# google/nerfies

Measured on NVIDIA H100. Metric: ray-samples/sec (coarse+fine, device-timed), higher is better.
Workload: dtype fp16x3 (fp32 emulated on wgmma: 3 fp16 MMA chains, fp32 accumulate)

## Files before the change

nerfies_b200/csrc/field_simt.cuh:

```cuda
#pragma once
#include "common.cuh"

namespace nfb {

constexpr int kTM = 64;
constexpr int kRS = kTM + 4;
constexpr int kKS = 16;
constexpr int kSimtThreads = 256;
constexpr int kSimtSmemFloats =
    2 * kMaxWidth * kRS
    + kMaxIn * kRS
    + 64 * kRS
    + 2 * kKS * kMaxWidth
    + 3 * kTM;
constexpr int kSimtSmemBytes = kSimtSmemFloats * 4;

constexpr int kDebugTimeout = 8, kDebugOneRowBlock = 16;

struct FieldArgs {
  const float* params;
  const float* origins;
  const float* directions;
  const float* z_vals;
  const float* points;
  const float* cond;
  const float* window;
  float* samples;
  float* warped;
  long long num_rows;
  int samples_per_ray;
  int use_warp;
  int warp_only;
  int debug;
  float* ray_out;
  float* ray_weights;
  int white_bg, sample_at_infinity;
};

__device__ __forceinline__ void cp_async16(void* smem, const void* gmem) {
  unsigned s = (unsigned)__cvta_generic_to_shared(smem);
  asm volatile("cp.async.cg.shared.global [%0], [%1], 16;\n" ::"r"(s), "l"(gmem));
}
__device__ __forceinline__ void cp_async_commit() {
  asm volatile("cp.async.commit_group;\n" ::);
}
template <int N>
__device__ __forceinline__ void cp_async_wait() {
  asm volatile("cp.async.wait_group %0;\n" ::"n"(N));
}

struct SimtSmem {
  float* buf[2];
  float* in;
  float* out;
  float* slab[2];
  float* wp;
  __device__ float* ptr(int id) const {
    return id == kB0 ? buf[0] : id == kB1 ? buf[1] : id == kOut0 ? out : out + 32 * kRS;
  }
// ... 189 lines not shown
```

nerfies_b200/csrc/field_tc.cuh:

```cuda
#pragma once
#include "field_simt.cuh"
#include "field_tc3.cuh"
#include "nfb_handle.h"
#include "tc_common.cuh"
#include "tc_program.cuh"

namespace nfb {
namespace tc {

__device__ __forceinline__ void posenc_fast_to_block(uint8_t* block, int r, const float* x, int F,
                                                  const float* __restrict__ window,
                                                  const float* __restrict__ extra, int n_extra,
                                                  int c_begin = 0, int c_end = 8) {
  float feat[64];
#pragma unroll
  for (int k = 0; k < 64; ++k) feat[k] = 0.f;
  float sn[3], cs[3];
#pragma unroll
  for (int c = 0; c < 3; ++c) {
    feat[c] = x[c];
    sincosf(x[c], &sn[c], &cs[c]);
  }
#pragma unroll
  for (int f = 0; f < 10; ++f) {
// ... 9 lines not shown
      }
    }
  }
  const int d = 3 + 6 * F;
#pragma unroll
  for (int k = 0; k < 64; ++k) {
    if (k >= d && k < d + n_extra) feat[k] = __ldg(extra + (k - d));
  }
#pragma unroll
  for (int c = 0; c < 8; ++c)
    if (c >= c_begin && c < c_end) store_chunk(block, r, c, feat + c * 8);
}
template <bool kX3, uint32_t kBlkBytes>
__device__ __forceinline__ void encode_input(uint8_t* in_block, int r, int hs, const float* x, int F,
                                             const float* __restrict__ window,
                                             const float* __restrict__ extra, int n_extra) {
  if constexpr (kX3) {
    if (hs == 0) tc3::posenc_block_x3<0>(in_block, in_block + kBlkBytes, r, x, F, window, extra, n_extra);
    else tc3::posenc_block_x3<1>(in_block, in_block + kBlkBytes, r, x, F, window, extra, n_extra);
  } else {
    posenc_fast_to_block(in_block, r, x, F, window, extra, n_extra, 4 * hs, 4 * hs + 4);
  }
}
__device__ __forceinline__ void cond_to_block(uint8_t* block, int r, const float* __restrict__ cond,
                                              int n, int c_begin = 0, int c_end = 8) {
#pragma unroll 1
  for (int c = c_begin; c < c_end; ++c) {
    float v[8];
#pragma unroll
    for (int j = 0; j < 8; ++j) {
      const int k = c * 8 + j;
      v[j] = k < n ? __ldg(cond + k) : 0.f;
    }
    store_chunk(block, r, c, v);
  }
}

template <bool kX3, uint32_t kBlkBytes>
__device__ __forceinline__ void epi_chunk(const float* acc, int c, const float* __restrict__ bias, float inv_s,
                                          bool relu, bool adot, const float* __restrict__ aw, float& al0,
                                          float& al1, uint8_t* act_hi, uint32_t* lo, int arow, int lq) {
#pragma unroll
  for (int j = 0; j < 16; ++j) {
    const int col = c * 128 + 8 * j + 2 * lq;
    const float2 b = __ldg(reinterpret_cast<const float2*>(bias + col));
    float v[4] = {fmaf(acc[4 * j], inv_s, b.x), fmaf(acc[4 * j + 1], inv_s, b.y),
                  fmaf(acc[4 * j + 2], inv_s, b.x), fmaf(acc[4 * j + 3], inv_s, b.y)};
    if (adot) {
      float2 w = __ldg(reinterpret_cast<const float2*>(aw + col));
      if constexpr (!kX3) w = __bfloat1622float2(__floats2bfloat162_rn(w.x, w.y));
      al0 = fmaf(relu ? fmaxf(v[0], 0.f) : v[0], w.x, al0);
      al0 = fmaf(relu ? fmaxf(v[1], 0.f) : v[1], w.y, al0);
      al1 = fmaf(relu ? fmaxf(v[2], 0.f) : v[2], w.x, al1);
      al1 = fmaf(relu ? fmaxf(v[3], 0.f) : v[3], w.y, al1);
    }
    const uint32_t blk = (uint32_t)(2 * c + (j >> 3)) * kBlkBytes + 4 * lq;
#pragma unroll
    for (int h = 0; h < 2; ++h) {
      const uint32_t off = blk + swz_off(arow + 8 * h, j & 7);
      const float a = v[2 * h], bb = v[2 * h + 1];
      uint32_t hi;
      if constexpr (kX3) {
        const float ta = __uint_as_float(__float_as_uint(a) & 0xFFFFE000u);
        const float tb = __uint_as_float(__float_as_uint(bb) & 0xFFFFE000u);
        const float da = a - ta, db = bb - tb;
        uint32_t& l = lo[x3_lo_reg(2 * c + (j >> 3), j & 7, h)];
        if (relu) {
          asm("cvt.rn.relu.satfinite.f16x2.f32 %0, %1, %2;" : "=r"(hi) : "f"(tb), "f"(ta));
          asm("cvt.rn.relu.satfinite.f16x2.f32 %0, %1, %2;" : "=r"(l) : "f"(db), "f"(da));
        } else {
          asm("cvt.rn.satfinite.f16x2.f32 %0, %1, %2;" : "=r"(hi) : "f"(tb), "f"(ta));
          asm("cvt.rn.satfinite.f16x2.f32 %0, %1, %2;" : "=r"(l) : "f"(db), "f"(da));
        }
      } else {
        if (relu) asm("cvt.rn.relu.bf16x2.f32 %0, %1, %2;" : "=r"(hi) : "f"(bb), "f"(a));
        else asm("cvt.rn.bf16x2.f32 %0, %1, %2;" : "=r"(hi) : "f"(bb), "f"(a));
      }
      *reinterpret_cast<uint32_t*>(act_hi + off) = hi;
    }
  }
}

template <bool kX3>
__device__ __noinline__ float alpha_cond_dot(const float* __restrict__ cond, const float* __restrict__ w, int n) {
  float a = 0.f;
  for (int j = 0; j < n; ++j) {
    float wj = __ldg(w + j);
    if constexpr (!kX3) wj = __bfloat162float(__float2bfloat16_rn(wj));
    a = fmaf(__ldg(cond + j), wj, a);
  }
  return a;
}

struct RowState {
  float x[3];
  long long m;
  long long ray;
  bool valid;
  float z, dist;
  bool last;
};

constexpr int kWgThreads = 384;
constexpr int kAlphaOff = 14 * kABlockBytes;
constexpr int kScanOff = kAlphaOff + 512;
constexpr int kBarOff = kScanOff + 256;
constexpr int kWgSmemBytes = kBarOff + 256;
template <bool kX3, int kMB>
struct WgSmem {
  static constexpr int kRows = kMB * kTileRows;
  static constexpr uint32_t kBlkBytes = kRows * kRowBytes;
  static constexpr int kSlots = (kX3 && kMB == 2) ? 3 : 4;
  static constexpr int kSlotBytes = (kX3 ? 2 : 1) * kABlockBytes;
  static constexpr int kRingOff = kAlphaOff - kSlots * kSlotBytes;
  static constexpr int kInOff = kRingOff - 2 * (int)kBlkBytes;
  static_assert(kInOff >= 4 * kABlockBytes, "input block overlaps the activation image");
};
static_assert(kWgSmemBytes <= 232448, "shared memory");

template <bool kX3, int N, int kActKb>
__device__ __forceinline__ void wg_layer_unit(float* d, int src, uint32_t a_hi, uint32_t in_lo, const uint32_t* lo,
                                              uint32_t b_hi, uint32_t b_lo, uint32_t accumulate) {
  if constexpr (kX3) {
    switch (src) {
      case 0: wg_unit<true, N>(d, a_hi, lo + x3_lo_reg(0, 0, 0), b_hi, b_lo, accumulate); break;
      case 1: wg_unit<true, N>(d, a_hi, lo + x3_lo_reg(1, 0, 0), b_hi, b_lo, accumulate); break;
      case 2:
        if constexpr (kActKb > 2) wg_unit<true, N>(d, a_hi, lo + x3_lo_reg(2, 0, 0), b_hi, b_lo, accumulate);
        break;
// ... 58 lines not shown
          const uint32_t bytes = (kX3 ? 2u : 1u) * (uint32_t)st.chunk_n * kRowBytes;
          const uint8_t* src = wpack + st.w_off;
          const int n = st.n_chunks * st.nkb;
          for (int u = 0; u < n; ++u) {
            mbar_wait(&bars->empty[sg], ph ^ 1, dead);
            if (!dead && elect_one()) {
              mbar_arrive_expect_tx(&bars->full[sg], bytes);
              bulk_g2s(ring + sg * kSlotBytes, src + (size_t)u * bytes, bytes, &bars->full[sg]);
            }
            __syncwarp();
            if (++sg == kSlots) { sg = 0; ph ^= 1; }
          }
        }
      }
    }
  } else {
    asm volatile("setmaxnreg.inc.sync.aligned.u32 %0;" ::"n"(kConsumerRegs));
    constexpr int kWgRows = 64 * kMB;
    const int cw = wg - 1, t = tid & 127, wq = t >> 5, lq = lane & 3;
    const int arow = kWgRows * cw + 16 * wq + (lane >> 2);
    const int lr = kMB == 2 ? t : (t & 63);
    const int r = kWgRows * cw + lr;
    const int h0 = kMB == 2 ? 0 : t >> 6, h1 = kMB == 2 ? 2 : h0 + 1;
    const int cb = h0 * 4, ce = cb + 4;
    uint8_t* act_hi = base;
    uint8_t* inh = base + Smem::kInOff;
    uint8_t* inl = inh + kBlk;
    float* alpha_s = reinterpret_cast<float*>(base + kAlphaOff);
    float* scan_s = reinterpret_cast<float*>(base + kScanOff);
    const uint32_t rows_off = (uint32_t)(kWgRows * cw * kRowBytes);
    float* scr = reinterpret_cast<float*>(base + rows_off);
    const uint32_t ring_a = smem_u32(base + Smem::kRingOff);
    const uint32_t act_a = smem_u32(act_hi) + rows_off, in_a = smem_u32(inh) + rows_off;
    uint32_t lo[kX3 ? 64 : 1];
    const float alpha_b = __ldg(aux + prog.alpha_b_off);
    const int S = args.samples_per_ray;
    uint32_t sg = 0, ph = 0, dead = 0;
    auto wg_sync = [&]() { asm volatile("bar.sync %0, 128;" ::"r"(1 + cw) : "memory"); };
    RowState row;

    auto begin_tile = [&](int tile) {
      long long m = (long long)tile * kRows + r;
      row.valid = m < args.num_rows;
      if (!row.valid) m = args.num_rows - 1;
      row.m = m;
      row.ray = m / S;
      const float z = args.z_vals ? __ldg(args.z_vals + m) : 0.f;
      float org[3], dir[3];
#pragma unroll
      for (int c = 0; c < 3; ++c) {
        dir[c] = __ldg(args.directions + row.ray * 3 + c);
        org[c] = __ldg(args.origins + row.ray * 3 + c);
      }
      if (args.points) {
#pragma unroll
        for (int c = 0; c < 3; ++c) row.x[c] = __ldg(args.points + m * 3 + c);
      } else {
#pragma unroll
        for (int c = 0; c < 3; ++c) row.x[c] = org[c] + z * dir[c];
      }
      if (fuse) {
        row.z = z;
        row.last = m + 1 == (row.ray + 1) * S;
        const float zn = (!row.last && args.z_vals) ? __ldg(args.z_vals + m + 1) : 0.f;
        const float dnorm = sqrtf(dir[0] * dir[0] + dir[1] * dir[1] + dir[2] * dir[2]);
        const float d = row.last ? (args.sample_at_infinity ? 1e10f : 1e-19f) : (zn - z);
        row.dist = d * dnorm;
      }
      if (!warp_pass && args.warped && row.valid && h0 == 0) {
// ... 41 lines not shown
            } else {
              wg_layer_unit<kX3, 128, kActKb>(acc0, src, a_hi, in_lo, lo, b_hi, b_lo, kb);
              wg_layer_unit<kX3, 128, kActKb>(acc1, src, a_hi + 8192u, in_lo + 8192u, lo + 32, b_hi, b_lo, kb);
            }
          }
          wg_commit();
          if (u > 0) {
            wg_wait<1>();
            if (lane == 0) mbar_arrive(&bars->empty[prev_sg]);
          }
          prev_sg = sg;
          if (++sg == kSlots) { sg = 0; ph ^= 1; }
        }
        wg_wait<0>();
        wg_fence_regs<64>(acc0); wg_fence_regs<64>(acc1);
        if (lane == 0) mbar_arrive(&bars->empty[prev_sg]);
        wg_sync();

        if (hidden) {
          const bool relu = st.relu != 0, adot = st.alpha_dot != 0;
          const float* aw = aux + prog.alpha_w_off;
          if constexpr (kMB == 1) {
            float al0 = 0.f, al1 = 0.f;
            epi_chunk<kX3, kBlk>(acc0, 0, bias, inv_s, relu, adot, aw, al0, al1, act_hi, lo, arow, lq);
            if (st.n_chunks == 2)
              epi_chunk<kX3, kBlk>(acc1, 1, bias, inv_s, relu, adot, aw, al0, al1, act_hi, lo, arow, lq);
            if (adot) {
              al0 += __shfl_xor_sync(0xffffffffu, al0, 1); al0 += __shfl_xor_sync(0xffffffffu, al0, 2);
              al1 += __shfl_xor_sync(0xffffffffu, al1, 1); al1 += __shfl_xor_sync(0xffffffffu, al1, 2);
              if (lq == 0) { alpha_s[arow] = al0; alpha_s[arow + 8] = al1; }
            }
            if (st.write_cond) {
              const float* cond = args.cond + row.ray * prog.cond_stride + prog.rc_off;
              if constexpr (kX3) tc3::cond_to_block_x3(inh, inl, r, cond, prog.rc, cb, ce);
              else cond_to_block(inh, r, cond, prog.rc, cb, ce);
            }
          } else {
            float al0 = 0.f, al1 = 0.f;
            epi_chunk<kX3, kBlk>(acc0, 0, bias, inv_s, relu, false, aw, al0, al1, act_hi, lo, arow, lq);
            epi_chunk<kX3, kBlk>(acc1, 0, bias, inv_s, relu, false, aw, al0, al1, act_hi, lo + 32, arow + 64, lq);
          }
        } else {
          const int l0 = 16 * wq + (lane >> 2);
#pragma unroll
          for (int b = 0; b < kMB; ++b) {
            const float* a16 = b == 0 ? acc0 : acc1;
#pragma unroll
            for (int h = 0; h < 2; ++h) {
              float* sr = scr + (l0 + 64 * b + 8 * h) * 16 + 2 * lq;
              sr[0] = a16[2 * h]; sr[1] = a16[2 * h + 1];
              sr[8] = a16[4 + 2 * h]; sr[9] = a16[5 + 2 * h];
            }
          }
          wg_sync();
          float v[12];
#pragma unroll
          for (int j = 0; j < 12; ++j) v[j] = fmaf(scr[lr * 16 + j], inv_s, __ldg(bias + j));
          wg_sync();
          if (st.epi == kEpiWarpHeads) {
            float y[3];
            warp_tail(prog.warp_type, v, row.x, prog.warp_pivot, prog.warp_trans, y);
            if (row.valid && h0 == 0) {
#pragma unroll
              for (int c = 0; c < 3; ++c) args.warped[row.m * 3 + c] = y[c];
            }
            if (has_next) begin_tile(tile_of(ti + 1));
          } else if constexpr (kMB == 1) {
            float4 o;
            o.x = sigmoidf(v[0]); o.y = sigmoidf(v[1]); o.z = sigmoidf(v[2]);
            const float a_cond = prog.ac ? alpha_cond_dot<kX3>(args.cond + row.ray * prog.cond_stride + prog.ac_off,
                                                               aux + prog.alpha_w_off + kAlphaCondOff, prog.ac)
                                         : 0.f;
            o.w = apply_act(alpha_b + (alpha_s[r] + a_cond), prog.sigma_act);
            if (h0 == 0 && row.valid && args.samples) reinterpret_cast<float4*>(args.samples)[row.m] = o;
            if (fuse && h0 == 0) {
              const int qd = r >> 5;
              auto bar128 = [&]() { asm volatile("bar.sync 3, 128;" ::: "memory"); };
              if ((tile % tpr) == 0) { c_T = 1.f; c_cw = 0.f; a_r = a_g = a_b = a_d = a_w = a_wnl = a_med = 0.f; }
              const float al = -expm1f(-o.w * row.dist);
              const float tf = 1.0f - al + 1e-10f;
              float P = tf;
#pragma unroll
              for (int sh = 1; sh < 32; sh <<= 1) {
                const float q = __shfl_up_sync(0xffffffffu, P, sh);
                if (lane >= sh) P = P * q;
              }
              float excl = __shfl_up_sync(0xffffffffu, P, 1);
              if (lane == 0) excl = 1.f;
              if (lane == 31) scan_s[qd] = P;
              bar128();
              float Wq = 1.f, Wall = 1.f;
#pragma unroll
              for (int q = 0; q < 4; ++q) {
                const float f = scan_s[q];
                if (q < qd) Wq = Wq * f;
                Wall = Wall * f;
// ... 43 lines not shown
                ro[5] = args.sample_at_infinity ? a_wnl : a_w;
              }
              bar128();
            }
            if (has_next) begin_tile(tile_of(ti + 1));
          }
          if constexpr (kX3) {
#pragma unroll
            for (int i = 0; i < 64; ++i) lo[i] = 0u;
          }
        }
        fence_proxy_async();
        wg_sync();
      }
    }
  }
  __syncthreads();
}

inline int tc_fail(const char* what) {
  return fail("the tensor-core paths (precision bf16 / fp16x3) do not support this model: %s; use precision fp32", what);
}

inline int build_tc_program(nfb_handle* h, int level, long long* wbytes, long long* aux_floats) {
  const FieldProgram& fp = h->prog[level];
  TcProgram& tp = h->tcprog[level];
  memset(&tp, 0, sizeof(tp));
  const int wparts = h->cfg.precision == NFB_PREC_FP16X3 ? 2 : 1;
  tp.warp_pivot = fp.warp_pivot; tp.warp_trans = fp.warp_trans;
  tp.warp_type = fp.warp_type; tp.Fw = fp.Fw; tp.G = fp.G; tp.Fp = fp.Fp; tp.rc = fp.rc;
  tp.cond_stride = fp.cond_stride; tp.sigma_act = fp.sigma_act;
  tp.tc = fp.tc; tp.ac = fp.ac; tp.ac_off = fp.G + fp.tc; tp.rc_off = fp.G + fp.tc + fp.ac;
  if (fp.rc > kBlockK) return tc_fail("rgb condition wider than 64 channels");
  if (fp.ac > kBlockK) return tc_fail("alpha condition wider than 64 channels");
  if (fp.Dp + fp.tc > kBlockK || (fp.warp_type && fp.Dw > kBlockK)) return tc_fail("encoded inputs wider than 64");
  if (fp.hidden_act != kRelu) return tc_fail("hidden activation other than relu");
  auto new_bias = [&](const Step& st) {
    int off = (int)*aux_floats;
    *aux_floats += 256;
    h->tc_aux_jobs.push_back({st.b_off, st.n, 1, off});
    return off;
  };
  auto add = [&](const Step& st, int epi, int cur_width) -> int {
    if (tp.n_steps >= kMaxTcSteps) return tc_fail("too many layers");
    TcStep& t = tp.steps[tp.n_steps];
    memset(&t, 0, sizeof(t));
    if (st.k_x > 256 || st.k_in > kBlockK) return tc_fail("layer wider than 256 or inputs wider than 64");
    if (st.k_x && st.k_x != cur_width) return tc_fail("unexpected layer input width");
    t.nkb = 0;
    if (st.k_in) t.src[t.nkb++] = kSrcIn;
    for (int b = 0; b < (st.k_x + kBlockK - 1) / kBlockK; ++b) t.src[t.nkb++] = b;
    t.epi = epi;
    if (epi == kEpiHidden) {
      if (st.n < 1 || st.n > 256) return tc_fail("hidden widths must be 1..256");
      t.n_chunks = (st.n + 127) / 128; t.chunk_n = 128;
      if (st.act != kRelu && st.act != kNone) return tc_fail("hidden activation other than relu");
      t.relu = st.act == kRelu;
    } else {
      t.n_chunks = 1; t.chunk_n = 16;
      if (st.n > 12) return tc_fail("head wider than 12");
      if (st.k_in) return tc_fail("head reading the encoded inputs");
    }
    t.b_off = new_bias(st);
    t.w_off = (uint32_t)*wbytes;
    for (int c = 0; c < t.n_chunks; ++c) {
      nfb_handle::TcPackJob job;
      job.level = level; job.step = tp.n_steps; job.chunk = c;
      job.simt_w_off = st.w_off; job.ld = st.npad; job.n = st.n; job.n0 = c * t.chunk_n;
      job.k_total = st.k_x + st.k_in;
      job.k_map.assign((size_t)t.nkb * kBlockK, -1);
      for (int kb = 0; kb < t.nkb; ++kb)
        for (int j = 0; j < kBlockK; ++j) {
          int srck = -1;
          if (t.src[kb] < kSrcIn) srck = t.src[kb] * kBlockK + j < st.k_x ? t.src[kb] * kBlockK + j : -1;
          else if (j < st.k_in) srck = st.k_x + j;
          job.k_map[(size_t)kb * kBlockK + j] = srck;
        }
      h->tc_jobs.push_back(job);
      *wbytes += (long long)wparts * t.nkb * t.chunk_n * kRowBytes;
    }
    ++tp.n_steps;
    return 0;
  };
  int width = 0;
  for (int i = 0; i < fp.warp.n_steps; ++i) {
    const Step& st = fp.warp.steps[i];
    const bool head = st.dst == kOut0 || st.dst == kOut1;
    if (add(st, head ? kEpiWarpHeads : kEpiHidden, width)) return -1;
    if (!head) width = st.n;
  }
  tp.n_warp = tp.n_steps;
  tp.warp_mb = 2;
  for (int i = 0; i < tp.n_warp; ++i)
    if (tp.steps[i].n_chunks != 1) tp.warp_mb = 1;
  width = 0;
  int last_hidden = -1;
  bool seen_alpha = false, seen_bottleneck = false;
  for (int i = 0; i < fp.nerf.n_steps; ++i) {
    const Step& st = fp.nerf.steps[i];
    if (st.dst == fp.alpha_slot && st.n == 1 && !seen_alpha) {
      if (st.k_in != fp.ac) return tc_fail("alpha head inputs");
      seen_alpha = true;
      const int src_step = (seen_bottleneck && !st.k_in) ? last_hidden - 1 : last_hidden;
      if (src_step < 0) return tc_fail("alpha head without a trunk layer");
      tp.steps[src_step].alpha_dot = 1;
      tp.alpha_w_off = (int)*aux_floats; *aux_floats += kAlphaCondOff + kBlockK;
      tp.alpha_b_off = (int)*aux_floats; *aux_floats += 4;
      h->tc_aux_jobs.push_back({st.w_off, st.k_x, st.npad, tp.alpha_w_off});
      if (st.k_in)
        h->tc_aux_jobs.push_back({st.w_off + st.k_x * st.npad, st.k_in, st.npad, tp.alpha_w_off + kAlphaCondOff});
      h->tc_aux_jobs.push_back({st.b_off, 1, 1, tp.alpha_b_off});
      continue;
    }
    const bool out = st.dst == fp.rgb_slot;
    if (!out && st.act == kNone) {
      seen_bottleneck = true;
    }
    if (add(st, out ? kEpiRgbOut : kEpiHidden, width)) return -1;
    if (!out) {
      last_hidden = tp.n_steps - 1;
      width = st.n;
      if (st.act == kNone) tp.steps[last_hidden].write_cond = 1;
    }
  }
  if (!seen_alpha) return tc_fail("model without alpha head");
  for (int si = 0; si < tp.n_steps; ++si) {
    const bool after_head = si > 0 && tp.steps[si - 1].epi != kEpiHidden;
    if ((si == 0 || after_head) && (tp.steps[si].nkb != 1 || tp.steps[si].src[0] != kSrcIn))
      return tc_fail("first layer of an MLP reading more than the encoded inputs");
  }
  tp.scale_off = (int)*aux_floats; *aux_floats += kMaxTcSteps;
  return 0;
}

inline int create_tc(nfb_handle* h) {
  long long wbytes = 0, auxf = 0;
  h->tc_jobs.clear(); h->tc_aux_jobs.clear();
  const int levels = h->cfg.num_fine_samples > 0 ? 2 : 1;
  for (int lv = 0; lv < levels; ++lv)
    if (build_tc_program(h, lv, &wbytes, &auxf)) return -1;
  if (levels == 1) h->tcprog[1] = h->tcprog[0];
  h->wpack_bytes = wbytes; h->aux_floats = auxf;
  if (cudaMalloc(&h->d_wpack, (size_t)wbytes) != cudaSuccess) return fail("cudaMalloc wpack failed");
  if (cudaMalloc(&h->d_aux, (size_t)auxf * sizeof(float)) != cudaSuccess) return fail("cudaMalloc aux failed");
  if (cudaMemset(h->d_aux, 0, (size_t)auxf * sizeof(float)) != cudaSuccess) return fail("cudaMemset failed");
  const auto smem_attr = cudaFuncAttributeMaxDynamicSharedMemorySize;
  if (cudaFuncSetAttribute(field_wg_kernel<true, 1>, smem_attr, kWgSmemBytes) != cudaSuccess ||
      cudaFuncSetAttribute(field_wg_kernel<true, 2>, smem_attr, kWgSmemBytes) != cudaSuccess ||
      cudaFuncSetAttribute(field_wg_kernel<false, 1>, smem_attr, kWgSmemBytes) != cudaSuccess ||
      cudaFuncSetAttribute(field_wg_kernel<false, 2>, smem_attr, kWgSmemBytes) != cudaSuccess)
    return fail("cannot reserve %d bytes of shared memory for the tensor-core kernel", kWgSmemBytes);
  return 0;
}

inline void destroy_tc(nfb_handle* h) {
  if (h->d_wpack) cudaFree(h->d_wpack);
  if (h->d_aux) cudaFree(h->d_aux);
  h->d_wpack = nullptr; h->d_aux = nullptr;
}

__global__ void aux_copy_kernel(const float* __restrict__ src, int count, int stride,
                                float* __restrict__ dst) {
  const int i = blockIdx.x * blockDim.x + threadIdx.x;
  if (i < count) dst[i] = src[(size_t)i * stride];
}

inline int pack_tc(nfb_handle* h, cudaStream_t s) {
  size_t total_map = 0;
  for (auto& j : h->tc_jobs) total_map += j.k_map.size();
  int* d_maps = nullptr;
  if (cudaMalloc(&d_maps, total_map * sizeof(int)) != cudaSuccess) return fail("cudaMalloc k_map failed");
  std::vector<int> all;
  all.reserve(total_map);
  for (auto& j : h->tc_jobs) all.insert(all.end(), j.k_map.begin(), j.k_map.end());
  cudaError_t e = cudaMemcpyAsync(d_maps, all.data(), total_map * sizeof(int), cudaMemcpyHostToDevice, s);
  if (e == cudaSuccess) e = cudaStreamSynchronize(s);
  if (e != cudaSuccess) { cudaFree(d_maps); return fail("k_map upload failed: %s", cudaGetErrorString(e)); }
  size_t map_off = 0;
  const bool x3 = h->cfg.precision == NFB_PREC_FP16X3;
  if (x3) {
    for (int lv = 0; lv < 2; ++lv)
      cudaMemsetAsync(h->d_aux + h->tcprog[lv].scale_off, 0, kMaxTcSteps * sizeof(float), s);
    for (auto& j : h->tc_jobs) {
      if (j.chunk != 0) continue;
      const long long n = (long long)j.k_total * j.ld;
      absmax_kernel<<<(unsigned)std::min<long long>((n + 255) / 256, 64), 256, 0, s>>>(
          h->d_packed + j.simt_w_off, n, h->d_aux + h->tcprog[j.level].scale_off + j.step);
      h->launches++;
    }
  }
  for (auto& j : h->tc_jobs) {
    const TcStep& t = h->tcprog[j.level].steps[j.step];
    const long long total = (long long)t.nkb * t.chunk_n * kBlockK;
    uint8_t* dst = h->d_wpack + t.w_off + (size_t)(x3 ? 2 : 1) * j.chunk * t.nkb * t.chunk_n * kRowBytes;
    if (x3)
      pack_weight_x3_kernel<<<(unsigned)((total + 255) / 256), 256, 0, s>>>(
          h->d_packed + j.simt_w_off + j.n0, j.ld, d_maps + map_off, t.nkb, j.n - j.n0, t.chunk_n,
          h->d_aux + h->tcprog[j.level].scale_off + j.step, dst);
    else
      pack_weight_kernel<<<(unsigned)((total + 255) / 256), 256, 0, s>>>(
          h->d_packed + j.simt_w_off + j.n0, j.ld, d_maps + map_off, t.nkb, j.n - j.n0, t.chunk_n,
          reinterpret_cast<__nv_bfloat16*>(dst));
    h->launches++;
    map_off += j.k_map.size();
  }
  for (auto& a : h->tc_aux_jobs) {
    aux_copy_kernel<<<(a.count + 127) / 128, 128, 0, s>>>(h->d_packed + a.src_off, a.count, a.stride,
                                                          h->d_aux + a.dst_off);
    h->launches++;
  }
  e = cudaGetLastError();
  if (e == cudaSuccess) e = cudaStreamSynchronize(s);
  cudaFree(d_maps);
  if (e != cudaSuccess) return fail("tensor-core weight packing failed: %s", cudaGetErrorString(e));
  return 0;
}

inline int run_field_tc(nfb_handle* h, int level, const FieldArgs& a, cudaStream_t s) {
  const TcProgram& prog = h->tcprog[level];
  if (a.warp_only && (prog.n_warp == 0 || !a.warped)) return fail("warp pass without a warp net or an output");
  if (!a.warp_only && a.use_warp && prog.n_warp > 0 && !a.points)
    return fail("the NeRF pass of a warped model needs the warp pass's points");
  const int mb = (a.warp_only && prog.warp_mb == 2 && !(a.debug & kDebugOneRowBlock)) ? 2 : 1;
  const long long rows_per_tile = (long long)mb * kTileRows;
  const long long tiles = (a.num_rows + rows_per_tile - 1) / rows_per_tile;
  if (tiles > 0x7fffffffLL) return fail("too many rows for one launch");
  const bool fuse = a.ray_out != nullptr && !a.warp_only;
  if (fuse && (a.samples_per_ray % kTileRows != 0 || a.num_rows % a.samples_per_ray != 0))
    return fail("fused composite needs samples_per_ray to be a multiple of %d", kTileRows);
  const long long groups = fuse ? a.num_rows / a.samples_per_ray : tiles;
  const int grid = (int)std::min<long long>(groups, h->sm_count);
  const bool x3 = h->cfg.precision == NFB_PREC_FP16X3;
  auto kernel = x3 ? (mb == 2 ? field_wg_kernel<true, 2> : field_wg_kernel<true, 1>)
                   : (mb == 2 ? field_wg_kernel<false, 2> : field_wg_kernel<false, 1>);
  kernel<<<grid, kWgThreads, kWgSmemBytes, s>>>(prog, a, h->d_wpack, h->d_aux, (int)tiles);
  cudaError_t e = cudaGetLastError();
  if (e != cudaSuccess) return fail("field_wg_kernel launch failed: %s", cudaGetErrorString(e));
  h->launches++;
  return 0;
}

}
// ... 2 lines not shown
```

nerfies_b200/csrc/field_tc3.cuh:

```cuda
#pragma once
#include <cuda_fp16.h>

#include "common.cuh"
#include "tc_common.cuh"

namespace nfb {
namespace tc3 {

using namespace nfb::tc;

__device__ __forceinline__ void split_pair(float a, float b, uint32_t& hi, uint32_t& lo) {
  asm("cvt.rn.satfinite.f16x2.f32 %0, %1, %2;" : "=r"(hi) : "f"(b), "f"(a));
  float fa, fb;
  asm("{\n\t.reg .f16 l, h;\n\tmov.b32 {l, h}, %2;\n\tcvt.f32.f16 %0, l;\n\tcvt.f32.f16 %1, h;\n\t}"
      : "=f"(fa), "=f"(fb) : "r"(hi));
  asm("cvt.rn.satfinite.f16x2.f32 %0, %1, %2;" : "=r"(lo) : "f"(b - fb), "f"(a - fa));
}

__device__ __forceinline__ void store_chunk_x3(uint8_t* bh, uint8_t* bl, int row, int chunk, const float* v) {
  uint4 qh, ql;
  split_pair(v[0], v[1], qh.x, ql.x);
  split_pair(v[2], v[3], qh.y, ql.y);
  split_pair(v[4], v[5], qh.z, ql.z);
  split_pair(v[6], v[7], qh.w, ql.w);
// ... 67 lines not shown
          const float t = a32[c] + kHalfPiF;
          const double eps = ((double)t - (double)a32[c]) - 1.57079632679489661923;
          const double v64 = fma(-sn[c], eps, fma(cs[c], -0.5 * eps * eps, cs[c]));
          const float v = (float)v64;
          feat[kc - 32 * kHS] = window ? w * v : v;
        }
        const double s2 = 2.0 * sn[c] * cs[c];
        const double c2 = fma(-2.0 * sn[c], sn[c], 1.0);
        sn[c] = s2; cs[c] = c2;
        a32[c] = a32[c] * 2.0f;
      }
    }
  }
  const int d = 3 + 6 * F;
#pragma unroll
  for (int j = 0; j < 32; ++j) {
    const int k = 32 * kHS + j;
    if (k >= d && k < d + n_extra) feat[j] = __ldg(extra + (k - d));
  }
#pragma unroll
  for (int c = 0; c < 4; ++c) store_chunk_x3(bh, bl, r, 4 * kHS + c, feat + 8 * c);
}

__device__ __forceinline__ void cond_to_block_x3(uint8_t* bh, uint8_t* bl, int r, const float* __restrict__ cond,
                                                 int n, int c_begin, int c_end) {
#pragma unroll 1
  for (int c = c_begin; c < c_end; ++c) {
    float v[8];
#pragma unroll
    for (int j = 0; j < 8; ++j) {
      const int k = c * 8 + j;
      v[j] = k < n ? __ldg(cond + k) : 0.f;
    }
    store_chunk_x3(bh, bl, r, c, v);
  }
}

}
}
```

nerfies_b200/csrc/nfb_handle.h:

```cpp
#pragma once
#include <cuda_runtime.h>

#include <cmath>
#include <cstdarg>
#include <cstdio>
#include <cstring>
#include <string>
#include <vector>

#include "../../include/nerfies_b200.h"
#include "common.cuh"
#include "ray_kernels.cuh"
#include "tc_program.cuh"

namespace {

thread_local std::string g_error;

int fail(const char* fmt, ...) {
  char buf[1024];
  va_list ap;
  va_start(ap, fmt);
  vsnprintf(buf, sizeof(buf), fmt, ap);
  va_end(ap);
// ... 54 lines not shown
  long long launches = 0;
  bool profiling = false;
  cudaEvent_t ev[2][2] = {{nullptr, nullptr}, {nullptr, nullptr}};
  bool ev_valid[2] = {false, false};
  nfb::CondLayout cond_layout{};
  int sm_count = 132;
  nfb::Net time_net{};
  float time_alpha = 0.f;
  cudaStream_t last_stream = nullptr;
  bool last_stream_valid = false;
  cudaEvent_t ev_order = nullptr;
  float* d_tape = nullptr; long long tape_floats = 0;
  float *d_gpacked = nullptr, *d_gwarp = nullptr, *d_gapp = nullptr, *d_gcam = nullptr;
  float *d_dcond = nullptr, *d_tr_out = nullptr, *d_tr_w = nullptr, *d_loss = nullptr;
  float* d_ttape = nullptr; long long ttape_floats = 0;
  float* d_time_tape = nullptr; long long time_tape_floats = 0;
  int* d_sel = nullptr; long long sel_cap = 0;
  int train_precision = NFB_TRAIN_FP32;
  int debug_bits = 0;
  nfb::tc::TcProgram tcprog[2];
  unsigned char* d_wpack = nullptr;
  float* d_aux = nullptr;
  long long wpack_bytes = 0, aux_floats = 0;
  struct TcPackJob { int level, step, chunk; int simt_w_off, ld, n, n0, k_total; std::vector<int> k_map; };
  std::vector<TcPackJob> tc_jobs;
  struct TcAuxJob { int src_off, count, stride, dst_off; };
  std::vector<TcAuxJob> tc_aux_jobs;
};
```

nerfies_b200/csrc/ray_kernels.cuh:

```cuda
#pragma once
#include <math_constants.h>

#include "../../include/nerfies_b200.h"
#include "common.cuh"

namespace nfb {

struct CondLayout {
  int G, tc, ac, dv, cc;
  int A, C;
  int stride;
  __host__ __device__ int rc() const { return dv + ac + cc; }
};

inline CondLayout cond_layout(const nfb_config& c) {
  CondLayout L{};
  L.G = c.warp_field_type != NFB_WARP_NONE ? c.num_warp_features : 0;
  L.A = c.num_appearance_features;
  L.C = c.num_camera_features;
  L.tc = (c.use_appearance_metadata && c.use_trunk_condition) ? L.A : 0;
  L.ac = (c.use_appearance_metadata && c.use_alpha_condition) ? L.A : 0;
  L.dv = c.use_viewdirs ? 3 + 6 * c.num_nerf_viewdir_freqs : 0;
  L.cc = c.use_camera_metadata ? L.C : 0;
  L.stride = L.G + L.tc + L.ac + L.rc();
// ... 40 lines not shown
__global__ void ray_cond_kernel(const CondArgs a) {
  const CondLayout& L = a.layout;
  const long long idx = (long long)blockIdx.x * blockDim.x + threadIdx.x;
  if (idx >= (long long)a.num_rays * L.stride) return;
  const int ray = (int)(idx / L.stride);
  int j;
  const CondSource src = cond_source(L, (int)(idx - (long long)ray * L.stride), j);
  auto embed = [&](const unsigned* ids, const float* table, int n, int width) {
    if (a.encoded && ids) return reinterpret_cast<const float*>(ids)[(size_t)ray * width + j];
    return table[embed_row(ids, ray, n) * width + j];
  };
  float v = 0.f;
  if (src == kCondWarp) {
    v = embed(a.warp_id, a.warp_table, a.n_warp, L.G);
  } else if (src == kCondApp) {
    v = embed(a.app_id, a.app_table, a.n_app, L.A);
  } else if (src == kCondCam) {
    v = embed(a.cam_id, a.cam_table, a.n_cam, L.C);
  } else if (src == kCondViewdir) {
    const float d[3] = {a.viewdirs[ray * 3 + 0], a.viewdirs[ray * 3 + 1], a.viewdirs[ray * 3 + 2]};
    v = (j < 3) ? d[j] : posenc_feature(d, j - 3);
  }
  a.cond[idx] = v;
}

constexpr int kTimeRays = 8;
constexpr int kTimeThreads = 128;
constexpr int kTimeMaxIn = 40;

__device__ __forceinline__ float time_encoding(float t, int k, const float* window) {
  if (k == 0) return t;
  const int f = (k - 1) >> 1, which = (k - 1) & 1;
  float ang = t * exp2f((float)f);
  if (which) ang = ang + kHalfPiF;
  return window[f] * sinf(ang);
}

struct TimeArgs {
  const float* params;
  Net net;
  const float* time_f;
  const unsigned* time_id;
  int F;
  float window[20];
  int blend;
  float time_alpha;
// ... 266 lines not shown
```

nerfies_b200/csrc/tc_program.cuh:

```cuda
#pragma once
#include <stdint.h>

namespace nfb {
namespace tc {

constexpr int kMaxTcSteps = 24;
constexpr int kSrcIn = 4;
constexpr int kAlphaCondOff = 256;

enum Epi { kEpiHidden = 0, kEpiWarpHeads = 1, kEpiRgbOut = 2 };

struct TcStep {
  uint32_t w_off;
  int nkb;
  int src[6];
  int n_chunks;
  int chunk_n;
  int b_off;
  int epi;
  int relu;
  int alpha_dot;
  int write_cond;
};

struct TcProgram {
  int n_steps;
  TcStep steps[kMaxTcSteps];
  int n_warp;
  int warp_mb;
  int warp_type, Fw, G, Fp, rc, cond_stride, sigma_act;
  int tc, ac;
  int ac_off, rc_off;
  int warp_pivot, warp_trans;
  int alpha_w_off, alpha_b_off;
  int scale_off;
};

}
}
```

Baseline: 128.9 million.

## Fold linear bottleneck layer into next layer and precompute per-ray condition bias

For the fp16x3 path, the linear (no-activation) bottleneck layer is algebraically folded into the following RGB hidden layer and into the alpha head, with the combined weights computed once in double precision at pack time. The condition-dependent part of that layer's input is turned into a per-ray bias vector (and a per-ray alpha offset) by a new small kernel launched before each field pass, so the tensor-core kernel skips one GEMM and the condition-to-block staging. This adds a kernel launch, a per-ray bias buffer read in the epilogue, and some fp32 rounding differences from the reassociated arithmetic.

```diff
diff --git a/nerfies_b200/csrc/field_simt.cuh b/nerfies_b200/csrc/field_simt.cuh
--- a/nerfies_b200/csrc/field_simt.cuh
+++ b/nerfies_b200/csrc/field_simt.cuh
@@ -35,6 +35,8 @@
   float* ray_out;
   float* ray_weights;
   int white_bg, sample_at_infinity;
+  const float* ray_bias;
+  const float* ray_alpha;
 };
 
 __device__ __forceinline__ void cp_async16(void* smem, const void* gmem) {
diff --git a/nerfies_b200/csrc/field_tc.cuh b/nerfies_b200/csrc/field_tc.cuh
--- a/nerfies_b200/csrc/field_tc.cuh
+++ b/nerfies_b200/csrc/field_tc.cuh
@@ -55,21 +55,8 @@
     posenc_fast_to_block(in_block, r, x, F, window, extra, n_extra, 4 * hs, 4 * hs + 4);
   }
 }
-__device__ __forceinline__ void cond_to_block(uint8_t* block, int r, const float* __restrict__ cond,
-                                              int n, int c_begin = 0, int c_end = 8) {
-#pragma unroll 1
-  for (int c = c_begin; c < c_end; ++c) {
-    float v[8];
-#pragma unroll
-    for (int j = 0; j < 8; ++j) {
-      const int k = c * 8 + j;
-      v[j] = k < n ? __ldg(cond + k) : 0.f;
-    }
-    store_chunk(block, r, c, v);
-  }
-}
-
-template <bool kX3, uint32_t kBlkBytes>
+
+template <bool kX3, uint32_t kBlkBytes, int kRows = 3>
 __device__ __forceinline__ void epi_chunk(const float* acc, int c, const float* __restrict__ bias, float inv_s,
                                           bool relu, bool adot, const float* __restrict__ aw, float& al0,
                                           float& al1, uint8_t* act_hi, uint32_t* lo, int arow, int lq) {
@@ -90,6 +77,7 @@
     const uint32_t blk = (uint32_t)(2 * c + (j >> 3)) * kBlkBytes + 4 * lq;
 #pragma unroll
     for (int h = 0; h < 2; ++h) {
+      if (!((kRows >> h) & 1)) continue;
       const uint32_t off = blk + swz_off(arow + 8 * h, j & 7);
       const float a = v[2 * h], bb = v[2 * h + 1];
       uint32_t hi;
@@ -114,14 +102,23 @@
   }
 }
 
-template <bool kX3>
+__device__ __forceinline__ void cond_to_block(uint8_t* block, int r, const float* __restrict__ cond,
+                                              int n, int c_begin, int c_end) {
+#pragma unroll 1
+  for (int c = c_begin; c < c_end; ++c) {
+    float v[8];
+#pragma unroll
+    for (int j = 0; j < 8; ++j) {
+      const int k = c * 8 + j;
+      v[j] = k < n ? __ldg(cond + k) : 0.f;
+    }
+    store_chunk(block, r, c, v);
+  }
+}
+
 __device__ __noinline__ float alpha_cond_dot(const float* __restrict__ cond, const float* __restrict__ w, int n) {
   float a = 0.f;
-  for (int j = 0; j < n; ++j) {
-    float wj = __ldg(w + j);
-    if constexpr (!kX3) wj = __bfloat162float(__float2bfloat16_rn(wj));
-    a = fmaf(__ldg(cond + j), wj, a);
-  }
+  for (int j = 0; j < n; ++j) a = fmaf(__ldg(cond + j), __bfloat162float(__float2bfloat16_rn(__ldg(w + j))), a);
   return a;
 }
 
@@ -137,7 +134,8 @@
 constexpr int kWgThreads = 384;
 constexpr int kAlphaOff = 14 * kABlockBytes;
 constexpr int kScanOff = kAlphaOff + 512;
-constexpr int kBarOff = kScanOff + 256;
+constexpr int kRayOff = kScanOff + 256;
+constexpr int kBarOff = kRayOff + 512;
 constexpr int kWgSmemBytes = kBarOff + 256;
 template <bool kX3, int kMB>
 struct WgSmem {
@@ -242,12 +240,11 @@
     const int lr = kMB == 2 ? t : (t & 63);
     const int r = kWgRows * cw + lr;
     const int h0 = kMB == 2 ? 0 : t >> 6, h1 = kMB == 2 ? 2 : h0 + 1;
-    const int cb = h0 * 4, ce = cb + 4;
     uint8_t* act_hi = base;
     uint8_t* inh = base + Smem::kInOff;
-    uint8_t* inl = inh + kBlk;
     float* alpha_s = reinterpret_cast<float*>(base + kAlphaOff);
     float* scan_s = reinterpret_cast<float*>(base + kScanOff);
+    int* ray_s = reinterpret_cast<int*>(base + kRayOff);
     const uint32_t rows_off = (uint32_t)(kWgRows * cw * kRowBytes);
     float* scr = reinterpret_cast<float*>(base + rows_off);
     const uint32_t ring_a = smem_u32(base + Smem::kRingOff);
@@ -265,6 +262,7 @@
       if (!row.valid) m = args.num_rows - 1;
       row.m = m;
       row.ray = m / S;
+      if (!warp_pass && h0 == 0) ray_s[r] = (int)row.ray;
       const float z = args.z_vals ? __ldg(args.z_vals + m) : 0.f;
       float org[3], dir[3];
 #pragma unroll
@@ -352,18 +350,29 @@
           const float* aw = aux + prog.alpha_w_off;
           if constexpr (kMB == 1) {
             float al0 = 0.f, al1 = 0.f;
-            epi_chunk<kX3, kBlk>(acc0, 0, bias, inv_s, relu, adot, aw, al0, al1, act_hi, lo, arow, lq);
-            if (st.n_chunks == 2)
-              epi_chunk<kX3, kBlk>(acc1, 1, bias, inv_s, relu, adot, aw, al0, al1, act_hi, lo, arow, lq);
+            if (kX3 && st.ray_bias) {
+              const int cols = 128 * st.n_chunks;
+              const float* rb = args.ray_bias + (size_t)ray_s[arow] * cols;
+              epi_chunk<kX3, kBlk, 1>(acc0, 0, rb, inv_s, relu, false, aw, al0, al1, act_hi, lo, arow, lq);
+              if (st.n_chunks == 2) epi_chunk<kX3, kBlk, 1>(acc1, 1, rb, inv_s, relu, false, aw, al0, al1, act_hi, lo, arow, lq);
+              rb = args.ray_bias + (size_t)ray_s[arow + 8] * cols;
+              epi_chunk<kX3, kBlk, 2>(acc0, 0, rb, inv_s, relu, false, aw, al0, al1, act_hi, lo, arow, lq);
+              if (st.n_chunks == 2) epi_chunk<kX3, kBlk, 2>(acc1, 1, rb, inv_s, relu, false, aw, al0, al1, act_hi, lo, arow, lq);
+            } else {
+              epi_chunk<kX3, kBlk>(acc0, 0, bias, inv_s, relu, adot, aw, al0, al1, act_hi, lo, arow, lq);
+              if (st.n_chunks == 2)
+                epi_chunk<kX3, kBlk>(acc1, 1, bias, inv_s, relu, adot, aw, al0, al1, act_hi, lo, arow, lq);
+            }
             if (adot) {
               al0 += __shfl_xor_sync(0xffffffffu, al0, 1); al0 += __shfl_xor_sync(0xffffffffu, al0, 2);
               al1 += __shfl_xor_sync(0xffffffffu, al1, 1); al1 += __shfl_xor_sync(0xffffffffu, al1, 2);
               if (lq == 0) { alpha_s[arow] = al0; alpha_s[arow + 8] = al1; }
             }
-            if (st.write_cond) {
-              const float* cond = args.cond + row.ray * prog.cond_stride + prog.rc_off;
-              if constexpr (kX3) tc3::cond_to_block_x3(inh, inl, r, cond, prog.rc, cb, ce);
-              else cond_to_block(inh, r, cond, prog.rc, cb, ce);
+            if constexpr (!kX3) {
+              if (st.write_cond) {
+                const float* cond = args.cond + row.ray * prog.cond_stride + prog.rc_off;
+                cond_to_block(inh, r, cond, prog.rc, 4 * h0, 4 * h0 + 4);
+              }
             }
           } else {
             float al0 = 0.f, al1 = 0.f;
@@ -398,10 +407,16 @@
           } else if constexpr (kMB == 1) {
             float4 o;
             o.x = sigmoidf(v[0]); o.y = sigmoidf(v[1]); o.z = sigmoidf(v[2]);
-            const float a_cond = prog.ac ? alpha_cond_dot<kX3>(args.cond + row.ray * prog.cond_stride + prog.ac_off,
-                                                               aux + prog.alpha_w_off + kAlphaCondOff, prog.ac)
-                                         : 0.f;
-            o.w = apply_act(alpha_b + (alpha_s[r] + a_cond), prog.sigma_act);
+            float a;
+            if constexpr (kX3) {
+              a = (prog.ac ? __ldg(args.ray_alpha + row.ray) : alpha_b) + alpha_s[r];
+            } else {
+              const float a_cond = prog.ac ? alpha_cond_dot(args.cond + row.ray * prog.cond_stride + prog.ac_off,
+                                                            aux + prog.alpha_w_off + kAlphaCondOff, prog.ac)
+                                           : 0.f;
+              a = alpha_b + (alpha_s[r] + a_cond);
+            }
+            o.w = apply_act(a, prog.sigma_act);
             if (h0 == 0 && row.valid && args.samples) reinterpret_cast<float4*>(args.samples)[row.m] = o;
             if (fuse && h0 == 0) {
               const int qd = r >> 5;
@@ -491,15 +506,19 @@
   return fail("the tensor-core paths (precision bf16 / fp16x3) do not support this model: %s; use precision fp32", what);
 }
 
-inline int build_tc_program(nfb_handle* h, int level, long long* wbytes, long long* aux_floats) {
+inline int build_tc_program(nfb_handle* h, int level, long long* wbytes, long long* aux_floats,
+                            long long* fold_floats) {
   const FieldProgram& fp = h->prog[level];
   TcProgram& tp = h->tcprog[level];
   memset(&tp, 0, sizeof(tp));
+  TcFold& fo = h->tc_fold[level];
+  memset(&fo, 0, sizeof(fo));
   const int wparts = h->cfg.precision == NFB_PREC_FP16X3 ? 2 : 1;
   tp.warp_pivot = fp.warp_pivot; tp.warp_trans = fp.warp_trans;
-  tp.warp_type = fp.warp_type; tp.Fw = fp.Fw; tp.G = fp.G; tp.Fp = fp.Fp; tp.rc = fp.rc;
+  tp.warp_type = fp.warp_type; tp.Fw = fp.Fw; tp.G = fp.G; tp.Fp = fp.Fp;
   tp.cond_stride = fp.cond_stride; tp.sigma_act = fp.sigma_act;
-  tp.tc = fp.tc; tp.ac = fp.ac; tp.ac_off = fp.G + fp.tc; tp.rc_off = fp.G + fp.tc + fp.ac;
+  tp.tc = fp.tc; tp.ac = fp.ac; tp.rc = fp.rc; tp.ac_off = fp.G + fp.tc; tp.rc_off = fp.G + fp.tc + fp.ac;
+  fo.ac_off = fp.G + fp.tc; fo.rc_off = fp.G + fp.tc + fp.ac;
   if (fp.rc > kBlockK) return tc_fail("rgb condition wider than 64 channels");
   if (fp.ac > kBlockK) return tc_fail("alpha condition wider than 64 channels");
   if (fp.Dp + fp.tc > kBlockK || (fp.warp_type && fp.Dw > kBlockK)) return tc_fail("encoded inputs wider than 64");
@@ -510,8 +529,9 @@
     h->tc_aux_jobs.push_back({st.b_off, st.n, 1, off});
     return off;
   };
-  auto add = [&](const Step& st, int epi, int cur_width) -> int {
-    if (tp.n_steps >= kMaxTcSteps) return tc_fail("too many layers");
+  int folded = 0;
+  auto add = [&](const Step& st, int epi, int cur_width, bool fold = false) -> int {
+    if (tp.n_steps + folded >= kMaxTcSteps) return tc_fail("too many layers");
     TcStep& t = tp.steps[tp.n_steps];
     memset(&t, 0, sizeof(t));
     if (st.k_x > 256 || st.k_in > kBlockK) return tc_fail("layer wider than 256 or inputs wider than 64");
@@ -530,13 +550,15 @@
       if (st.n > 12) return tc_fail("head wider than 12");
       if (st.k_in) return tc_fail("head reading the encoded inputs");
     }
-    t.b_off = new_bias(st);
+    if (fold) t.ray_bias = 1;
+    else t.b_off = new_bias(st);
     t.w_off = (uint32_t)*wbytes;
     for (int c = 0; c < t.n_chunks; ++c) {
       nfb_handle::TcPackJob job;
       job.level = level; job.step = tp.n_steps; job.chunk = c;
       job.simt_w_off = st.w_off; job.ld = st.npad; job.n = st.n; job.n0 = c * t.chunk_n;
       job.k_total = st.k_x + st.k_in;
+      job.fold = fold;
       job.k_map.assign((size_t)t.nkb * kBlockK, -1);
       for (int kb = 0; kb < t.nkb; ++kb)
         for (int j = 0; j < kBlockK; ++j) {
@@ -562,34 +584,65 @@
   tp.warp_mb = 2;
   for (int i = 0; i < tp.n_warp; ++i)
     if (tp.steps[i].n_chunks != 1) tp.warp_mb = 1;
+  const bool fold = h->cfg.precision == NFB_PREC_FP16X3;
   width = 0;
   int last_hidden = -1;
-  bool seen_alpha = false, seen_bottleneck = false;
+  bool seen_alpha = false, fold_pending = false, seen_bottleneck = false;
   for (int i = 0; i < fp.nerf.n_steps; ++i) {
     const Step& st = fp.nerf.steps[i];
     if (st.dst == fp.alpha_slot && st.n == 1 && !seen_alpha) {
       if (st.k_in != fp.ac) return tc_fail("alpha head inputs");
       seen_alpha = true;
-      const int src_step = (seen_bottleneck && !st.k_in) ? last_hidden - 1 : last_hidden;
+      const int src_step = (!fold && seen_bottleneck && !st.k_in) ? last_hidden - 1 : last_hidden;
       if (src_step < 0) return tc_fail("alpha head without a trunk layer");
       tp.steps[src_step].alpha_dot = 1;
       tp.alpha_w_off = (int)*aux_floats; *aux_floats += kAlphaCondOff + kBlockK;
       tp.alpha_b_off = (int)*aux_floats; *aux_floats += 4;
-      h->tc_aux_jobs.push_back({st.w_off, st.k_x, st.npad, tp.alpha_w_off});
-      if (st.k_in)
-        h->tc_aux_jobs.push_back({st.w_off + st.k_x * st.npad, st.k_in, st.npad, tp.alpha_w_off + kAlphaCondOff});
-      h->tc_aux_jobs.push_back({st.b_off, 1, 1, tp.alpha_b_off});
+      if (st.k_in && !fold) {
+        h->tc_aux_jobs.push_back({st.w_off, st.k_x, st.npad, tp.alpha_w_off, false});
+        h->tc_aux_jobs.push_back({st.w_off + st.k_x * st.npad, st.k_in, st.npad, tp.alpha_w_off + kAlphaCondOff, false});
+      } else if (st.k_in) {
+        fo.ac = st.k_in; fo.lda = st.npad; fo.wa = st.w_off; fo.ba = st.b_off;
+        h->tc_aux_jobs.push_back({fo.fwa, st.k_x, 1, tp.alpha_w_off, true});
+      } else {
+        h->tc_aux_jobs.push_back({st.w_off, st.k_x, st.npad, tp.alpha_w_off, false});
+      }
+      h->tc_aux_jobs.push_back({st.b_off, 1, 1, tp.alpha_b_off, false});
       continue;
     }
     const bool out = st.dst == fp.rgb_slot;
+    if (!out && st.act == kNone && !fold) {
+      seen_bottleneck = true;
+      if (add(st, kEpiHidden, width)) return -1;
+      last_hidden = tp.n_steps - 1;
+      tp.steps[last_hidden].write_cond = 1;
+      continue;
+    }
     if (!out && st.act == kNone) {
-      seen_bottleneck = true;
+      fo.active = 1; fo.W = st.n; fo.ldb = st.npad; fo.wb = st.w_off; fo.bb = st.b_off;
+      fo.fwa = (int)*fold_floats; fo.fca = fo.fwa + (fo.W + 3) / 4 * 4; fo.fc = fo.fca + 4; fo.fw = fo.fc + 256;
+      *fold_floats = fo.fw;
+      ++folded;
+      fold_pending = true;
+      continue;
+    }
+    if (fold_pending) {
+      fold_pending = false;
+      if (out) return tc_fail(st.k_in ? "head reading the encoded inputs" : "rgb logit reading the bottleneck");
+      fo.nr = st.n; fo.ldr = st.npad; fo.rc = st.k_in; fo.wr = st.w_off; fo.br = st.b_off;
+      fo.cols = 128 * ((st.n + 127) / 128);
+      *fold_floats += (long long)fo.W * fo.ldr;
+      Step f = st;
+      f.k_in = 0; f.w_off = fo.fw;
+      if (add(f, kEpiHidden, width, true)) return -1;
+      last_hidden = tp.n_steps - 1;
+      width = st.n;
+      continue;
     }
     if (add(st, out ? kEpiRgbOut : kEpiHidden, width)) return -1;
     if (!out) {
       last_hidden = tp.n_steps - 1;
       width = st.n;
-      if (st.act == kNone) tp.steps[last_hidden].write_cond = 1;
     }
   }
   if (!seen_alpha) return tc_fail("model without alpha head");
@@ -603,16 +656,22 @@
 }
 
 inline int create_tc(nfb_handle* h) {
-  long long wbytes = 0, auxf = 0;
+  long long wbytes = 0, auxf = 0, foldf = 0;
   h->tc_jobs.clear(); h->tc_aux_jobs.clear();
   const int levels = h->cfg.num_fine_samples > 0 ? 2 : 1;
   for (int lv = 0; lv < levels; ++lv)
-    if (build_tc_program(h, lv, &wbytes, &auxf)) return -1;
-  if (levels == 1) h->tcprog[1] = h->tcprog[0];
+    if (build_tc_program(h, lv, &wbytes, &auxf, &foldf)) return -1;
+  if (levels == 1) { h->tcprog[1] = h->tcprog[0]; h->tc_fold[1] = h->tc_fold[0]; }
   h->wpack_bytes = wbytes; h->aux_floats = auxf;
   if (cudaMalloc(&h->d_wpack, (size_t)wbytes) != cudaSuccess) return fail("cudaMalloc wpack failed");
   if (cudaMalloc(&h->d_aux, (size_t)auxf * sizeof(float)) != cudaSuccess) return fail("cudaMalloc aux failed");
   if (cudaMemset(h->d_aux, 0, (size_t)auxf * sizeof(float)) != cudaSuccess) return fail("cudaMemset failed");
+  if (h->tc_fold[0].active) {
+    const size_t rb = (size_t)h->max_rays * (h->tc_fold[0].cols + 1);
+    if (cudaMalloc(&h->d_fold, (size_t)foldf * sizeof(float)) != cudaSuccess ||
+        cudaMalloc(&h->d_ray_bias, rb * sizeof(float)) != cudaSuccess)
+      return fail("cudaMalloc of the bottleneck fold buffers failed");
+  }
   const auto smem_attr = cudaFuncAttributeMaxDynamicSharedMemorySize;
   if (cudaFuncSetAttribute(field_wg_kernel<true, 1>, smem_attr, kWgSmemBytes) != cudaSuccess ||
       cudaFuncSetAttribute(field_wg_kernel<true, 2>, smem_attr, kWgSmemBytes) != cudaSuccess ||
@@ -625,13 +684,32 @@
 inline void destroy_tc(nfb_handle* h) {
   if (h->d_wpack) cudaFree(h->d_wpack);
   if (h->d_aux) cudaFree(h->d_aux);
-  h->d_wpack = nullptr; h->d_aux = nullptr;
+  if (h->d_fold) cudaFree(h->d_fold);
+  if (h->d_ray_bias) cudaFree(h->d_ray_bias);
+  h->d_wpack = nullptr; h->d_aux = nullptr; h->d_fold = nullptr; h->d_ray_bias = nullptr;
 }
 
 __global__ void aux_copy_kernel(const float* __restrict__ src, int count, int stride,
                                 float* __restrict__ dst) {
   const int i = blockIdx.x * blockDim.x + threadIdx.x;
   if (i < count) dst[i] = src[(size_t)i * stride];
+}
+
+__global__ void fold_kernel(const float* __restrict__ p, const TcFold f, float* __restrict__ out) {
+  const int idx = blockIdx.x * blockDim.x + threadIdx.x;
+  const int cols = f.ldr + 1;
+  if (idx >= (f.W + 1) * cols) return;
+  const int i = idx / cols, j = idx - i * cols;
+  const bool alpha = j == f.ldr, bias = i == f.W;
+  if (alpha && !f.ac) return;
+  float* o = alpha ? out + (bias ? f.fca : f.fwa + i) : out + (bias ? f.fc : f.fw + i * f.ldr) + j;
+  if (!alpha && j >= f.nr) { *o = 0.f; return; }
+  const float* x = bias ? p + f.bb : p + f.wb + (size_t)i * f.ldb;
+  const float* y = alpha ? p + f.wa : p + f.wr + j;
+  const int ldy = alpha ? f.lda : f.ldr;
+  double v = bias ? (double)p[alpha ? f.ba : f.br + j] : 0.0;
+  for (int k = 0; k < f.W; ++k) v = fma((double)x[k], (double)y[(size_t)k * ldy], v);
+  *o = (float)v;
 }
 
 inline int pack_tc(nfb_handle* h, cudaStream_t s) {
@@ -647,6 +725,14 @@
   if (e != cudaSuccess) { cudaFree(d_maps); return fail("k_map upload failed: %s", cudaGetErrorString(e)); }
   size_t map_off = 0;
   const bool x3 = h->cfg.precision == NFB_PREC_FP16X3;
+  for (int lv = 0; lv < (h->cfg.num_fine_samples > 0 ? 2 : 1); ++lv) {
+    const TcFold& f = h->tc_fold[lv];
+    if (!f.active) continue;
+    const int n = (f.W + 1) * (f.ldr + 1);
+    fold_kernel<<<(n + 127) / 128, 128, 0, s>>>(h->d_packed, f, h->d_fold);
+    h->launches++;
+  }
+  auto src = [&](bool fold) { return fold ? h->d_fold : h->d_packed; };
   if (x3) {
     for (int lv = 0; lv < 2; ++lv)
       cudaMemsetAsync(h->d_aux + h->tcprog[lv].scale_off, 0, kMaxTcSteps * sizeof(float), s);
@@ -654,7 +740,7 @@
       if (j.chunk != 0) continue;
       const long long n = (long long)j.k_total * j.ld;
       absmax_kernel<<<(unsigned)std::min<long long>((n + 255) / 256, 64), 256, 0, s>>>(
-          h->d_packed + j.simt_w_off, n, h->d_aux + h->tcprog[j.level].scale_off + j.step);
+          src(j.fold) + j.simt_w_off, n, h->d_aux + h->tcprog[j.level].scale_off + j.step);
       h->launches++;
     }
   }
@@ -664,17 +750,17 @@
     uint8_t* dst = h->d_wpack + t.w_off + (size_t)(x3 ? 2 : 1) * j.chunk * t.nkb * t.chunk_n * kRowBytes;
     if (x3)
       pack_weight_x3_kernel<<<(unsigned)((total + 255) / 256), 256, 0, s>>>(
-          h->d_packed + j.simt_w_off + j.n0, j.ld, d_maps + map_off, t.nkb, j.n - j.n0, t.chunk_n,
+          src(j.fold) + j.simt_w_off + j.n0, j.ld, d_maps + map_off, t.nkb, j.n - j.n0, t.chunk_n,
           h->d_aux + h->tcprog[j.level].scale_off + j.step, dst);
     else
       pack_weight_kernel<<<(unsigned)((total + 255) / 256), 256, 0, s>>>(
-          h->d_packed + j.simt_w_off + j.n0, j.ld, d_maps + map_off, t.nkb, j.n - j.n0, t.chunk_n,
+          src(j.fold) + j.simt_w_off + j.n0, j.ld, d_maps + map_off, t.nkb, j.n - j.n0, t.chunk_n,
           reinterpret_cast<__nv_bfloat16*>(dst));
     h->launches++;
     map_off += j.k_map.size();
   }
   for (auto& a : h->tc_aux_jobs) {
-    aux_copy_kernel<<<(a.count + 127) / 128, 128, 0, s>>>(h->d_packed + a.src_off, a.count, a.stride,
+    aux_copy_kernel<<<(a.count + 127) / 128, 128, 0, s>>>(src(a.fold) + a.src_off, a.count, a.stride,
                                                           h->d_aux + a.dst_off);
     h->launches++;
   }
@@ -685,8 +771,26 @@
   return 0;
 }
 
-inline int run_field_tc(nfb_handle* h, int level, const FieldArgs& a, cudaStream_t s) {
+inline int run_field_tc(nfb_handle* h, int level, const FieldArgs& args, cudaStream_t s) {
   const TcProgram& prog = h->tcprog[level];
+  FieldArgs a = args;
+  const TcFold& f = h->tc_fold[level];
+  if (!a.warp_only && f.active && a.num_rows > 0) {
+    RayBiasArgs r{};
+    r.num_rays = (int)((a.num_rows + a.samples_per_ray - 1) / a.samples_per_ray);
+    r.cond = a.cond; r.stride = prog.cond_stride;
+    r.w_rc = h->d_packed + f.wr + (size_t)f.W * f.ldr; r.ldr = f.ldr; r.rc = f.rc; r.rc_off = f.rc_off;
+    r.c_r = h->d_fold + f.fc; r.nr = f.nr; r.cols = f.cols;
+    r.w_ac = h->d_packed + f.wa + (size_t)f.W * f.lda; r.lda = f.lda; r.ac = f.ac; r.ac_off = f.ac_off;
+    r.c_a = h->d_fold + f.fca;
+    r.bias = h->d_ray_bias; r.alpha = h->d_ray_bias + (size_t)h->max_rays * f.cols;
+    const long long n = (long long)r.num_rays * (f.cols + (f.ac > 0));
+    ray_bias_kernel<<<(unsigned)((n + 255) / 256), 256, 0, s>>>(r);
+    cudaError_t e = cudaGetLastError();
+    if (e != cudaSuccess) return fail("ray_bias_kernel launch failed: %s", cudaGetErrorString(e));
+    h->launches++;
+    a.ray_bias = r.bias; a.ray_alpha = r.alpha;
+  }
   if (a.warp_only && (prog.n_warp == 0 || !a.warped)) return fail("warp pass without a warp net or an output");
   if (!a.warp_only && a.use_warp && prog.n_warp > 0 && !a.points)
     return fail("the NeRF pass of a warped model needs the warp pass's points");
diff --git a/nerfies_b200/csrc/field_tc3.cuh b/nerfies_b200/csrc/field_tc3.cuh
--- a/nerfies_b200/csrc/field_tc3.cuh
+++ b/nerfies_b200/csrc/field_tc3.cuh
@@ -113,19 +113,5 @@
   for (int c = 0; c < 4; ++c) store_chunk_x3(bh, bl, r, 4 * kHS + c, feat + 8 * c);
 }
 
-__device__ __forceinline__ void cond_to_block_x3(uint8_t* bh, uint8_t* bl, int r, const float* __restrict__ cond,
-                                                 int n, int c_begin, int c_end) {
-#pragma unroll 1
-  for (int c = c_begin; c < c_end; ++c) {
-    float v[8];
-#pragma unroll
-    for (int j = 0; j < 8; ++j) {
-      const int k = c * 8 + j;
-      v[j] = k < n ? __ldg(cond + k) : 0.f;
-    }
-    store_chunk_x3(bh, bl, r, c, v);
-  }
-}
-
 }
 }
diff --git a/nerfies_b200/csrc/nfb_handle.h b/nerfies_b200/csrc/nfb_handle.h
--- a/nerfies_b200/csrc/nfb_handle.h
+++ b/nerfies_b200/csrc/nfb_handle.h
@@ -100,8 +100,11 @@
   unsigned char* d_wpack = nullptr;
   float* d_aux = nullptr;
   long long wpack_bytes = 0, aux_floats = 0;
-  struct TcPackJob { int level, step, chunk; int simt_w_off, ld, n, n0, k_total; std::vector<int> k_map; };
+  struct TcPackJob { int level, step, chunk; int simt_w_off, ld, n, n0, k_total; bool fold; std::vector<int> k_map; };
   std::vector<TcPackJob> tc_jobs;
-  struct TcAuxJob { int src_off, count, stride, dst_off; };
+  struct TcAuxJob { int src_off, count, stride, dst_off; bool fold; };
   std::vector<TcAuxJob> tc_aux_jobs;
+  nfb::tc::TcFold tc_fold[2];
+  float* d_fold = nullptr;
+  float* d_ray_bias = nullptr;
 };
diff --git a/nerfies_b200/csrc/ray_kernels.cuh b/nerfies_b200/csrc/ray_kernels.cuh
--- a/nerfies_b200/csrc/ray_kernels.cuh
+++ b/nerfies_b200/csrc/ray_kernels.cuh
@@ -86,6 +86,41 @@
     v = (j < 3) ? d[j] : posenc_feature(d, j - 3);
   }
   a.cond[idx] = v;
+}
+
+struct RayBiasArgs {
+  const float* cond;
+  int stride, num_rays;
+  const float* w_rc;
+  int ldr, rc, rc_off, nr, cols;
+  const float* c_r;
+  const float* w_ac;
+  int lda, ac, ac_off;
+  const float* c_a;
+  float* bias;
+  float* alpha;
+};
+
+__global__ void ray_bias_kernel(const RayBiasArgs a) {
+  const int per = a.cols + (a.ac > 0);
+  const long long idx = (long long)blockIdx.x * blockDim.x + threadIdx.x;
+  if (idx >= (long long)a.num_rays * per) return;
+  const long long ray = idx / per;
+  const int j = (int)(idx - ray * per);
+  const float* cond = a.cond + ray * a.stride;
+  if (j < a.cols) {
+    double v = 0.0;
+    if (j < a.nr) {
+      v = (double)a.c_r[j];
+      for (int q = 0; q < a.rc; ++q)
+        v = fma((double)cond[a.rc_off + q], (double)a.w_rc[(size_t)q * a.ldr + j], v);
+    }
+    a.bias[ray * a.cols + j] = (float)v;
+  } else {
+    double v = (double)a.c_a[0];
+    for (int q = 0; q < a.ac; ++q) v = fma((double)cond[a.ac_off + q], (double)a.w_ac[(size_t)q * a.lda], v);
+    a.alpha[ray] = (float)v;
+  }
 }
 
 constexpr int kTimeRays = 8;
diff --git a/nerfies_b200/csrc/tc_program.cuh b/nerfies_b200/csrc/tc_program.cuh
--- a/nerfies_b200/csrc/tc_program.cuh
+++ b/nerfies_b200/csrc/tc_program.cuh
@@ -20,6 +20,7 @@
   int epi;
   int relu;
   int alpha_dot;
+  int ray_bias;
   int write_cond;
 };
 
@@ -36,5 +37,16 @@
   int scale_off;
 };
 
+struct TcFold {
+  int active;
+  int W, ldb;
+  int nr, ldr, rc;
+  int cols;
+  int lda, ac;
+  int rc_off, ac_off;
+  int wb, bb, wr, br, wa, ba;
+  int fw, fc, fwa, fca;
+};
+
 }
 }
```

Measured after the change: 142.8 million (median of 6 runs). +10.8%, better.
